# ADVRHumanoids/OpenSoT

Measured on AMD Instinct MI355X. Metric: whole-body QP solves/sec (32-DoF, 3-level stack), higher is better.
Workload: dtype f64

## Files before the change

opensot_amd/csrc/osot_host_plan.h:

```cpp
#pragma once
#include "osot_plan_shape.h"
#include "osot_kernels.h"

namespace osot {

inline int pick_np(int n) {
#ifdef OSOT_X_NO_NP40
    return (n <= 32) ? 32 : ((n <= WaveCtx<56>::NMAX) ? 56 : 64);
#else
    return (n <= 32) ? 32 : ((n <= WaveCtx<40>::NMAX) ? 40 : ((n <= WaveCtx<56>::NMAX) ? 56 : 64));
#endif
}
inline int wave_lds_doubles(int NP) {
    return NP == 32 ? WaveCtx<32>::LDS_DOUBLES : (NP == 40 ? WaveCtx<40>::LDS_DOUBLES : (NP == 56 ? WaveCtx<56>::LDS_DOUBLES : WaveCtx<64>::LDS_DOUBLES));
}

inline int lds_layout(int NP, int n_rows, int* rows_off, int* rows_cap) {
    int d = (wave_lds_doubles(NP) + 1) & ~1;
    *rows_off = d;
    const int cap = ((n_rows > 0 ? n_rows : 1) + 1) & ~1;
    *rows_cap = cap;
    d += row_table_doubles(cap);
    d = (d + 1) & ~1;
    return d;
}

inline int make_dev_plan(const osot_plan_desc& p, const unsigned char* level_active, DevPlan& P, int& NP,
                         size_t& lds_bytes, const unsigned char* task_active = nullptr) {
    std::memset(&P, 0, sizeof(P));
    make_plan_shape(p, level_active, task_active, P);
    for (int k = 0; k < p.n_levels; ++k) P.ident_rows[k] = P.m[k] - P.ma[k];
    NP = pick_np(p.n);
    const int nrows_max = P.nc + P.optoff[p.n_levels];
    const int cap = ((nrows_max > 0 ? nrows_max : 1) + 1) & ~1;
    int total = (wave_lds_doubles(NP) + 1) & ~1;
    P.lds_rows_off = total;
    P.lds_rows_cap = cap;
    const int table = row_table_doubles(cap);
    P.rows_doubles = table;
    P.rows_in_global = 0;
    if (NP > 32) {
        const size_t with = (size_t)(total + table) * sizeof(double), without = (size_t)total * sizeof(double);
        if ((160 * 1024) / without > (160 * 1024) / with) P.rows_in_global = 1;
    }
    if (!P.rows_in_global) total += table;
    lds_bytes = (size_t)total * sizeof(double);
    return OSOT_OK;
}

inline void make_update_plan(const osot_plan_desc& pl, DevUpdatePlan& U) {
    std::memset(&U, 0, sizeof(U));
    U.n = pl.n; U.L = pl.n_levels;
    plan_constraint_rows(&pl, &U.nc);
    plan_stored_constraint_rows(&pl, &U.nc_stored);
    int flat = 0;
    for (int k = 0; k < pl.n_levels; ++k) {
        plan_level_rows(&pl, k, &U.m[k], &U.ma[k]);
        int off = 0;
        for (int j = 0; j < pl.level[k].n_tasks; ++j) {
            const osot_task_desc& t = pl.level[k].task[j];
            DevTaskS& d = U.task[flat++];
            d.level = k; d.kind = t.kind; d.rows = t.rows; d.off = off;
            d.weight = t.weight; d.lambda = t.lambda; d.ogain = t.orientation_gain; d.lambda2 = t.lambda2;
            d.mask = t.row_mask; d.prow = task_parent_rows(t, pl.n); d.sublam = t.row_mask ? t.sub_lambda : 1.0;
            d.gains = t.acc_gain_matrices ? 1 : 0;
            d.body = t.body_frame; d.dense = t.dense_weight;
            if (t.dense_weight) U.dense_level[k] = 1;
            off += t.rows;
        }
    }
    if (pl.has_regularisation) {
        const osot_task_desc& t = pl.regularisation;
        DevTaskS& d = U.task[flat++];
        d.level = -1; d.kind = t.kind; d.rows = t.rows; d.off = 0;
        d.weight = t.weight; d.lambda = t.lambda; d.ogain = t.orientation_gain; d.lambda2 = t.lambda2;
        d.mask = 0ull; d.prow = t.rows; d.sublam = 1.0;
        d.gains = 0; d.body = 0; d.dense = 0;
    }
    U.ntasks = flat;
    {
        int fr = 0;
        for (int j = 0; j < flat; ++j)
            for (int r = 0; r < U.task[j].rows && fr < OSOT_KMAX_FLAT_ROWS; ++r, ++fr) { U.row_task[fr] = (unsigned char)j; U.row_in_task[fr] = (short)r; }
        U.total_rows = fr;
        for (int k = 0; k < pl.n_levels; ++k) if (U.dense_level[k]) U.any_dense = 1;
    }
    U.nbounds = pl.n_bounds;
    for (int j = 0; j < pl.n_bounds; ++j) {
        U.bound[j].kind = pl.bound[j].kind; U.bound[j].scaling = pl.bound[j].scaling; U.bound[j].dT = pl.bound[j].dT;
    }
    U.nrowblocks = pl.n_rowblocks;
    int roff = 0, soff = 0;
    for (int j = 0; j < pl.n_rowblocks; ++j) {
        const osot_rows_desc& r = pl.rowblock[j];
        DevRowBlockS& d = U.rowblock[j];
        d.kind = r.kind; d.rows = r.rows; d.off = roff; d.stored_off = soff; d.first_col = r.first_col;
        d.body = r.task_body_frame; d.ncand = r.n_candidates;
        d.dT = r.dT; d.p = r.p; d.mu = r.mu; d.lambda = r.task_lambda; d.ogain = r.task_orientation_gain;
        for (int i = 0; i < OSOT_MAX_BAND_ROWS; ++i) { d.err_lb[i] = r.err_lb[i]; d.err_ub[i] = r.err_ub[i]; }
        d.d_threshold = r.d_threshold; d.detection_threshold = r.detection_threshold; d.bound_scaling = r.bound_scaling;
        if (!rows_are_implicit(d.kind)) soff += d.rows;
        roff += d.rows;
    }
}

inline int make_update_args(const osot_plan_desc& pl, const DevUpdatePlan& PL, const osot_leaf_batch* leaf,
                            const osot_assembled_out* out, const DevUpdatePlan* dev_plan, DevUpdate& U, const char** why) {
    std::memset(&U, 0, sizeof(U));
    U.B = leaf->B;
    U.plan = dev_plan;
    int flat = 0;
    for (int k = 0; k < pl.n_levels; ++k) {
        if (!out->b[k]) { *why = "out.b[k] is null"; return OSOT_ERR_INVALID; }
        U.b[k] = out->b[k]; U.w[k] = out->w[k];
        if (PL.dense_level[k]) {
            if (!out->WA[k] || !out->Wb[k] || (PL.ma[k] > 0 && !out->A[k]))
                { *why = "level has a non-diagonal weight: out.WA[k], out.Wb[k] and out.A[k] are required"; return OSOT_ERR_INVALID; }
            U.WA[k] = out->WA[k]; U.Wb[k] = out->Wb[k]; U.A[k] = out->A[k];
        }
        for (int j = 0; j < pl.level[k].n_tasks; ++j) {
            const osot_task_desc& t = pl.level[k].task[j];
            DevPtr4& d = U.task[flat++];
            d.p0 = leaf->task[k][j].p0; d.p1 = leaf->task[k][j].p1; d.p2 = leaf->task[k][j].p2; d.W = leaf->task[k][j].W;
            if (!d.p0) { *why = "leaf input p0 of a task is null"; return OSOT_ERR_INVALID; }
            if (t.kind != OSOT_TASK_GENERIC && t.kind != OSOT_TASK_ACC_POSTURAL && !d.p1)
                { *why = "leaf input p1 of a task is null"; return OSOT_ERR_INVALID; }
            if (t.dense_weight && !d.W) { *why = "task has dense_weight but its leaf W is null"; return OSOT_ERR_INVALID; }
        }
    }
    if (pl.has_regularisation) {
        const osot_task_desc& t = pl.regularisation;
        if (!out->b_reg) { *why = "out.b_reg is null"; return OSOT_ERR_INVALID; }
        DevPtr4& d = U.task[flat++];
        d.p0 = leaf->regularisation.p0; d.p1 = leaf->regularisation.p1; d.p2 = leaf->regularisation.p2; d.W = nullptr;
        if (!d.p0) { *why = "leaf input p0 of the regularisation task is null"; return OSOT_ERR_INVALID; }
        if (t.kind == OSOT_TASK_POSTURAL && !d.p1) { *why = "leaf input p1 of the regularisation task is null"; return OSOT_ERR_INVALID; }
        U.b_reg = out->b_reg;
    }
    for (int j = 0; j < pl.n_bounds; ++j) {
        DevPtr3& d = U.bound[j];
        const int kind = pl.bound[j].kind;
        d.p0 = leaf->bound[j].p0; d.p1 = leaf->bound[j].p1; d.p2 = leaf->bound[j].p2;
        if (!d.p0) { *why = "leaf input p0 of a bound is null"; return OSOT_ERR_INVALID; }
        if (kind == OSOT_BOUND_JOINT_LIMITS && (!d.p1 || !d.p2)) { *why = "joint limits need q, q_min, q_max"; return OSOT_ERR_INVALID; }
        if (kind == OSOT_BOUND_GENERIC && !d.p1) { *why = "generic bound needs l and u"; return OSOT_ERR_INVALID; }
    }
    if (pl.n_bounds > 0 && (!out->l || !out->u)) { *why = "out.l/out.u is null"; return OSOT_ERR_INVALID; }
    U.l = out->l; U.u = out->u;
    for (int j = 0; j < pl.n_rowblocks; ++j) {
        DevPtr3& d = U.rows[j];
        const int kind = pl.rowblock[j].kind;
        d.p0 = leaf->rows[j].p0; d.p1 = leaf->rows[j].p1; d.p2 = leaf->rows[j].p2;
        if (!d.p0) { *why = "leaf input p0 of a row block is null"; return OSOT_ERR_INVALID; }
        if ((kind == OSOT_ROWS_GENERIC || kind == OSOT_ROWS_COLLISION || kind == OSOT_ROWS_TORQUE_LIMITS ||
             kind == OSOT_ROWS_ACC_JOINT_LIMITS || kind == OSOT_ROWS_ACC_VELOCITY_LIMITS ||
             kind == OSOT_ROWS_TASK_CARTESIAN || kind == OSOT_ROWS_TASK_COM || kind == OSOT_ROWS_UNIT_GENERIC) && !d.p1)
            { *why = "leaf input p1 of a row block is null"; return OSOT_ERR_INVALID; }
        if (kind == OSOT_ROWS_ACC_JOINT_LIMITS && !d.p2) { *why = "acceleration joint limits need qddot_max"; return OSOT_ERR_INVALID; }
        if (kind == OSOT_ROWS_GENERIC && !d.p2) { *why = "generic rows need C, lo, up"; return OSOT_ERR_INVALID; }
        if ((kind == OSOT_ROWS_COP || kind == OSOT_ROWS_NORMAL_TORQUE) && !d.p1)
            { *why = "CoP / normal torque rows need the contact's x / y limits (p1)"; return OSOT_ERR_INVALID; }
    }
    if (PL.nc > 0 && (!out->lo || !out->up)) { *why = "out.lo/up is null"; return OSOT_ERR_INVALID; }
    if (PL.nc_stored > 0 && !out->C) { *why = "out.C is null"; return OSOT_ERR_INVALID; }
    U.C = out->C; U.lo = out->lo; U.up = out->up;
    return OSOT_OK;
}

}
```

opensot_amd/csrc/osot_kernels.h:

```cpp
#pragma once
#include "osot_plan_shape.h"
#include "osot_qp_core.h"

#ifndef OSOT_WAVES32
#define OSOT_WAVES32 2
#endif
#ifndef OSOT_WAVES40
#define OSOT_WAVES40 2
#endif

namespace osot {

struct DevPlan {
    int n, L, nc;
    int m[OSOT_KMAX_LEVELS];
    int ma[OSOT_KMAX_LEVELS];
    int optoff[OSOT_KMAX_LEVELS + 1];
    int ident_rows[OSOT_KMAX_LEVELS];
    int nblocks, nc_stored;
    int blk_rows[OSOT_KMAX_ROWBLOCKS], blk_off[OSOT_KMAX_ROWBLOCKS], blk_stored_off[OSOT_KMAX_ROWBLOCKS];
    int blk_implicit[OSOT_KMAX_ROWBLOCKS], blk_first_col[OSOT_KMAX_ROWBLOCKS];
    int blk_level[OSOT_KMAX_ROWBLOCKS];
    int max_iter;
    unsigned active_mask;
    int ntask[OSOT_KMAX_LEVELS];
    int task_off[OSOT_KMAX_LEVELS][OSOT_KMAX_TASKS + 1];
    unsigned inactive[OSOT_KMAX_LEVELS];
    double eps_abs;
    int reg_rows;
    double reg_w;
    int reg_dense;
    int lds_rows_off;
    int lds_rows_cap;
    int rows_doubles;
    int rows_in_global;
};

struct DevBatch {
    int B;
    const double* A[OSOT_KMAX_LEVELS];
    const double* b[OSOT_KMAX_LEVELS];
    const double* w[OSOT_KMAX_LEVELS];
    const double* c[OSOT_KMAX_LEVELS];
    const double* C;
    const double* lo;
    const double* up;
    const double* l;
    const double* u;
    double* dq;
    double* x_levels;
    int* status;
    int* iterations;
    long long* prof;
    const int* order;
    int* cost_out;
    const int* cost_in;
    int* order_next;
    int slots;
    const double* b_reg;
    const double* A_reg;
    const double* WA[OSOT_KMAX_LEVELS];
    const double* Wb[OSOT_KMAX_LEVELS];
    double* accepted_slack;
    double* rows_scratch;
    int* hot;
};
static_assert(std::is_trivially_copyable<DevPlan>::value && std::is_trivially_copyable<DevBatch>::value, "kernel arguments, zeroed with memset");

template <int NP, bool PROF, bool EXTRA, bool BOX = false>
__device__ __forceinline__ void cascade_body(const DevPlan& P, const DevBatch& D, const long long inst, const int lane, char* osot_smem) {
    constexpr int HV = WaveCtx<NP>::HV, S = WaveCtx<NP>::S;
    constexpr int HB = (NP % 16 == 0) ? 16 : 8;
    const int n = P.n;
    double* base = reinterpret_cast<double*>(osot_smem);
    WaveCtx<NP> w;
    w.c = WaveCtx<NP>::col_of(lane); w.h = WaveCtx<NP>::half_of(lane); w.n = n;
    w.M1 = base;
    w.M2 = base + WaveCtx<NP>::M1_DOUBLES;
    w.V = w.M2 + WaveCtx<NP>::ROWS * S;
    if constexpr (NP == 32) w.rlo = base + P.lds_rows_off;
    else w.rlo = P.rows_in_global ? D.rows_scratch + inst * P.rows_doubles : base + P.lds_rows_off;
    w.rup = w.rlo + P.lds_rows_cap;
    w.rptr = reinterpret_cast<unsigned long long*>(w.rup + P.lds_rows_cap);
    w.rowstate = reinterpret_cast<int*>(w.rptr + P.lds_rows_cap);
    w.eqlist = w.rowstate + P.lds_rows_cap;
    w.safe_row = reinterpret_cast<unsigned long long>(D.dq + inst * n);
    w.rsrc = reinterpret_cast<signed char*>(w.eqlist + P.lds_rows_cap);
    const int c = w.c, h = w.h;
    const bool valid = c < n;
    for (int e = lane; e < WaveCtx<NP>::LDS_DOUBLES; e += 64) base[e] = 0.0;
    wave_sync();

    const bool has_box = D.l != nullptr;
    double lb = (has_box && valid) ? D.l[inst * n + c] : -INFINITY;
    double ub = (has_box && valid) ? D.u[inst * n + c] : INFINITY;

    for (int j = 0; j < P.nblocks; ++j) {
        for (int q = lane; q < P.blk_rows[j]; q += 64) {
            const int r = P.blk_off[j] + q;
            w.rlo[r] = clamp_inf(D.lo[inst * P.nc + r]);
            w.rup[r] = clamp_inf(D.up[inst * P.nc + r]);
            w.rptr[r] = P.blk_implicit[j]
                ? ((((unsigned long long)(P.blk_first_col[j] + q)) << 1) | 1ull)
                : reinterpret_cast<unsigned long long>(D.C + (inst * P.nc_stored + P.blk_stored_off[j] + q) * n);
            w.rsrc[r] = -1;
        }
    }
    wave_sync();

    const bool regd = EXTRA && P.reg_dense && D.b_reg != nullptr;
    const bool regc = D.b_reg != nullptr && !regd && c < P.reg_rows;
    const double greg = regc ? -P.reg_w * D.b_reg[inst * P.reg_rows + c] : 0.0;
    const double dreg = regc ? P.reg_w : 0.0;

    double x = 0.0;
    int status = QP_SOLVED;
    int iters_total = 0;
    bool any = false;
    double slack = 0.0;
    long long prof[PH_COUNT];
    if (PROF) for (int i = 0; i < PH_COUNT; ++i) prof[i] = 0;
    const long long t_begin = PROF ? (long long)clock64() : 0;
    for (int k = 0; k < P.L; ++k) {
        if (!((P.active_mask >> k) & 1u)) {
            if (k + 1 < P.L) {
                const int off = P.nc + P.optoff[k];
                for (int q = lane; q < P.m[k]; q += 64) {
                    w.rlo[off + q] = -kInfty; w.rup[off + q] = kInfty; w.rptr[off + q] = (0x7fffffffull << 1) | 1ull;
                    w.rsrc[off + q] = -1;
                }
                wave_sync();
            }
            continue;
        }
        for (int j = 0; j < P.nblocks; ++j) {
            if (P.blk_level[j] == 0) continue;
            const bool on = P.blk_level[j] - 1 == k;
            for (int q = lane; q < P.blk_rows[j]; q += 64) {
                const int r = P.blk_off[j] + q;
                w.rlo[r] = on ? clamp_inf(D.lo[inst * P.nc + r]) : -kInfty;
                w.rup[r] = on ? clamp_inf(D.up[inst * P.nc + r]) : kInfty;
                w.rsrc[r] = on ? -2 : -1;
            }
            wave_sync();
        }
        OSOT_PH_BEGIN();
        {
            const int l2 = launder_i(lane);
            w.c = WaveCtx<NP>::col_of(l2); w.h = WaveCtx<NP>::half_of(l2);
        }
        const int c = w.c, h = w.h;
        const bool valid = c < n;
        const int m = P.m[k], ma = P.ma[k];
// ... 456 lines not shown
    const int h0 = hist[4 * lane], h1 = hist[4 * lane + 1], h2 = hist[4 * lane + 2], h3 = hist[4 * lane + 3];
    const int tot = h0 + h1 + h2 + h3;
    int v = tot;
#pragma unroll
    for (int off = 1; off < 64; off <<= 1) {
        const int t = __shfl_down(v, off, 64);
        v += (lane + off < 64) ? t : 0;
    }
    const int above = v - tot;
    start[4 * lane + 3] = above;
    start[4 * lane + 2] = above + h3;
    start[4 * lane + 1] = above + h3 + h2;
    start[4 * lane] = above + h3 + h2 + h1;
    __syncthreads();
    const int late = B - slots;
    const bool paired = late > 0 && B < 2 * slots;
    for (int i = lane; i < B; i += 64) {
        const int pos = __hip_atomic_fetch_add(&start[key(i)], 1, __ATOMIC_RELAXED, __HIP_MEMORY_SCOPE_WORKGROUP);
        int where = pos;
        if (paired) {
            const int alone = slots - late;
            if (pos >= B - late) where = alone + (B - 1 - pos);
            else if (pos >= alone) where = slots + (pos - alone);
        }
        order[where] = i;
    }
}
#else
inline void order_body(const int*, int*, int, int, int, char*) {}
#endif

__device__ __forceinline__ long long dispatch_instance(const DevBatch& D, char* smem) {
    int g = (int)blockIdx.x;
    if (D.order_next) {
        if (g == 0) { order_body(D.cost_in, D.order_next, D.B, D.slots, (int)threadIdx.x, smem); return -1; }
        g -= 1;
    }
    if (D.order) wave_priority_by_rank((unsigned)g, (unsigned)D.B);
    return D.order ? D.order[g] : g;
}

struct DevQP {
    int B, n, nc, max_iter;
    double eps_abs;
    const double* H;
    const double* g;
    const double* A;
    const double* lA;
    const double* uA;
    const double* l;
    const double* u;
    double* x;
    int* status;
    int* iterations;
    int lds_rows_off, lds_rows_cap;
    int* hot;
};

template <int NP, bool HOT = false>
__global__ void __launch_bounds__(64, (NP == 40 ? OSOT_WAVES40 : 1)) osot_qp_kernel(const DevQP Q) {
    OSOT_DYNAMIC_LDS(osot_smem);
    constexpr int S = WaveCtx<NP>::S;
    const int lane = threadIdx.x;
    const long long inst = blockIdx.x;
    const int n = Q.n;
    double* base = reinterpret_cast<double*>(osot_smem);
    WaveCtx<NP> w;
    w.c = WaveCtx<NP>::col_of(lane); w.h = WaveCtx<NP>::half_of(lane); w.n = n;
    w.M1 = base; w.M2 = base + WaveCtx<NP>::M1_DOUBLES; w.V = w.M2 + WaveCtx<NP>::ROWS * S;
    w.rlo = base + Q.lds_rows_off;
    w.rup = w.rlo + Q.lds_rows_cap;
    w.rptr = reinterpret_cast<unsigned long long*>(w.rup + Q.lds_rows_cap);
    w.rowstate = reinterpret_cast<int*>(w.rptr + Q.lds_rows_cap);
    w.eqlist = w.rowstate + Q.lds_rows_cap;
    w.safe_row = reinterpret_cast<unsigned long long>(Q.x + inst * n);
    w.rsrc = reinterpret_cast<signed char*>(w.eqlist + Q.lds_rows_cap);
    const int c = w.c, h = w.h;
    const bool valid = c < n;
    for (int e = lane; e < WaveCtx<NP>::LDS_DOUBLES; e += 64) base[e] = 0.0;
    wave_sync();
    constexpr int HV = WaveCtx<NP>::HV;
    double Hc[NP / HV];
    if constexpr (NP == 32) {
        const int ta = lane & 15, tq = lane >> 4;
#pragma unroll
        for (int t = 0; t < 16; ++t) {
            const int i = 16 * (t >> 3) + tq + 4 * (t & 3), cc = 16 * ((t >> 2) & 1) + ta;
            Hc[t] = (i < n && cc < n) ? Q.H[(inst * n + i) * n + cc] + ((i == cc) ? Q.eps_abs : 0.0)
                                      : ((i == cc) ? 1.0 : 0.0);
        }
    } else if constexpr (kWideTiles) {
        constexpr int T = wide_tiles(NP);
        const int ta = lane & 15, tq = lane >> 4;
#pragma unroll
        for (int I = 0; I < T; ++I)
#pragma unroll
            for (int C2 = I; C2 < T; ++C2)
#pragma unroll
                for (int r = 0; r < 4; ++r) {
                    const int i = 16 * I + tq + 4 * r, cc = 16 * C2 + ta;
                    Hc[4 * tile_u<T>(I, C2) + r] = (i < n && cc < n) ? Q.H[(inst * n + i) * n + cc] + ((i == cc) ? Q.eps_abs : 0.0)
                                                                      : ((i == cc) ? 1.0 : 0.0);
                }
    } else {
#pragma unroll
        for (int ii = 0; ii < NP / HV; ++ii) {
            const int i = HV * ii + h;
            Hc[ii] = (valid && i < n) ? Q.H[(inst * n + i) * n + c] + ((i == c) ? Q.eps_abs : 0.0)
                                      : ((i == c) ? 1.0 : 0.0);
        }
    }
    wave_sync();
    const double g = valid ? Q.g[inst * n + c] : 0.0;
    const bool has_box = Q.l != nullptr;
    double lb = (has_box && valid) ? Q.l[inst * n + c] : -INFINITY;
    double ub = (has_box && valid) ? Q.u[inst * n + c] : INFINITY;
    for (int r = lane; r < Q.nc; r += 64) {
        w.rlo[r] = clamp_inf(Q.lA[inst * Q.nc + r]);
        w.rup[r] = clamp_inf(Q.uA[inst * Q.nc + r]);
        w.rptr[r] = reinterpret_cast<unsigned long long>(Q.A + (inst * Q.nc + r) * n);
        w.rsrc[r] = -1;
    }
    wave_sync();
    double x = 0.0, slack = 0.0;
    int iters = 0;
    int st;
    int* hotk = (HOT && Q.hot) ? Q.hot + inst * WaveCtx<NP>::LW : nullptr;
    const int hotcode = hotk ? hotk[c] : -1;
    if (NP > 32) {
        OSOT_ALWAYS_INLINE_CALL st = gi_solve<NP, false>(w, Q.nc, g, false, 0.0, Hc, has_box, lb, ub, Q.max_iter, false, 0.0, x, iters, nullptr, slack,
                                                         false, 0.0, hotcode, hotk);
    } else {
        st = gi_solve<NP, false>(w, Q.nc, g, false, 0.0, Hc, has_box, lb, ub, Q.max_iter, false, 0.0, x, iters, nullptr, slack,
                                 false, 0.0, hotcode, hotk);
    }
    if (valid && h == 0) Q.x[inst * n + c] = (st == QP_SOLVED) ? x : 0.0;
    if (lane == 0) {
        Q.status[inst] = st;
        if (Q.iterations) Q.iterations[inst] = iters;
    }
}

struct DevTaskS {
    int level, kind, rows, off, prow, body, dense, gains;
    double weight, lambda, ogain, lambda2, sublam;
    unsigned long long mask;
};
struct DevBoundS { int kind; double scaling, dT; };
struct DevRowBlockS {
    int kind, rows, off, stored_off, first_col, body, ncand;
    double d_threshold, detection_threshold, bound_scaling, dT, p, mu, lambda, ogain;
    double err_lb[OSOT_MAX_BAND_ROWS], err_ub[OSOT_MAX_BAND_ROWS];
};
struct DevUpdatePlan {
    int n, L, nc, nc_stored;
    int m[OSOT_KMAX_LEVELS], ma[OSOT_KMAX_LEVELS];
    int dense_level[OSOT_KMAX_LEVELS];
    int any_dense;
    int total_rows;
    unsigned char row_task[OSOT_KMAX_FLAT_ROWS];
    short row_in_task[OSOT_KMAX_FLAT_ROWS];
    int ntasks;
    DevTaskS task[OSOT_KMAX_FLAT_TASKS];
    int nbounds;
    DevBoundS bound[OSOT_KMAX_BOUNDS];
    int nrowblocks;
    DevRowBlockS rowblock[OSOT_KMAX_ROWBLOCKS];
};
struct DevPtr4 { const double *p0, *p1, *p2, *W; };
struct DevPtr3 { const double *p0, *p1, *p2; };
struct DevUpdate {
    int B;
    const DevUpdatePlan* plan;
    DevPtr4 task[OSOT_KMAX_FLAT_TASKS];
    DevPtr3 bound[OSOT_KMAX_BOUNDS];
    DevPtr3 rows[OSOT_KMAX_ROWBLOCKS];
    double* b[OSOT_KMAX_LEVELS];
    double* w[OSOT_KMAX_LEVELS];
    double* WA[OSOT_KMAX_LEVELS];
    double* Wb[OSOT_KMAX_LEVELS];
    const double* A[OSOT_KMAX_LEVELS];
    double* C;
    double* lo;
    double* up;
    double* l;
    double* u;
    double* b_reg;
};
static_assert(sizeof(DevUpdate) <= 4096, "kernel arguments are limited to 4 KB");
static_assert(sizeof(DevUpdate) % 16 == 0 && sizeof(DevUpdatePlan) % 16 == 0, "staged into LDS in 16-byte pieces");
constexpr int kUpdateLdsBytes = (int)sizeof(DevUpdate) + (int)sizeof(DevUpdatePlan) + 256 * 8 + 258 * 4 + 8;

__device__ inline void rot_to_quat(const double* R, double* q) {
    double t = R[0] + R[4] + R[8];
    if (t > 0.0) {
        t = sqrt(t + 1.0);
        q[3] = 0.5 * t;
        t = 0.5 / t;
        q[0] = (R[7] - R[5]) * t;
        q[1] = (R[2] - R[6]) * t;
        q[2] = (R[3] - R[1]) * t;
    } else {
        int i = 0;
        if (R[4] > R[0]) i = 1;
        if (R[8] > ((i == 1) ? R[4] : R[0])) i = 2;
        if (i == 0) {
            t = sqrt(R[0] - R[4] - R[8] + 1.0);
            q[0] = 0.5 * t;
            t = 0.5 / t;
            q[3] = (R[7] - R[5]) * t;
            q[1] = (R[3] + R[1]) * t;
            q[2] = (R[6] + R[2]) * t;
        } else if (i == 1) {
            t = sqrt(R[4] - R[8] - R[0] + 1.0);
            q[1] = 0.5 * t;
            t = 0.5 / t;
            q[3] = (R[2] - R[6]) * t;
            q[2] = (R[7] + R[5]) * t;
            q[0] = (R[1] + R[3]) * t;
        } else {
            t = sqrt(R[8] - R[0] - R[4] + 1.0);
            q[2] = 0.5 * t;
            t = 0.5 / t;
            q[3] = (R[3] - R[1]) * t;
            q[0] = (R[2] + R[6]) * t;
            q[1] = (R[5] + R[7]) * t;
        }
    }
}

__device__ inline void cartesian_b(const double* Ta, const double* Td, const double* twist,
                                   double lambda, double ogain, double* b6, bool body = false) {
    double q[4], qd[4];
    rot_to_quat(Ta, q);
    rot_to_quat(Td, qd);
    const double dot = q[0] * qd[0] + q[1] * qd[1] + q[2] * qd[2] + q[3] * qd[3];
    const double sg = (dot < 0.0) ? -1.0 : 1.0;
    const double qx = sg * q[0], qy = sg * q[1], qz = sg * q[2], qw = sg * q[3];
    double eo[3];
    eo[0] = qd[3] * qx - qw * qd[0] + (-qd[2] * qy + qd[1] * qz);
    eo[1] = qd[3] * qy - qw * qd[1] + (qd[2] * qx - qd[0] * qz);
    eo[2] = qd[3] * qz - qw * qd[2] + (-qd[1] * qx + qd[0] * qy);
    for (int i = 0; i < 3; ++i) {
        const double tw_p = twist ? twist[i] : 0.0, tw_o = twist ? twist[3 + i] : 0.0;
        b6[i] = tw_p + lambda * (Td[9 + i] - Ta[9 + i]);
        b6[3 + i] = tw_o + lambda * (-ogain * eo[i]);
    }
    if (body) {
        double r6[6];
        for (int i = 0; i < 3; ++i) {
            r6[i] = Ta[i] * b6[0] + Ta[3 + i] * b6[1] + Ta[6 + i] * b6[2];
            r6[3 + i] = Ta[i] * b6[3] + Ta[3 + i] * b6[4] + Ta[6 + i] * b6[5];
        }
        for (int i = 0; i < 6; ++i) b6[i] = r6[i];
    }
}

__device__ inline double wrench_row_entry(int kind, int rr, int col, const double* R, const double* lim, double mu) {
    double a[6] = {0.0, 0.0, 0.0, 0.0, 0.0, 0.0};
    if (kind == 10) {
        const double m = mu / sqrt(2.0);
        a[0] = (rr == 0) ? 1.0 : (rr == 1 ? -1.0 : 0.0);
        a[1] = (rr == 2) ? 1.0 : (rr == 3 ? -1.0 : 0.0);
        a[2] = (rr == 4) ? -1.0 : -m;
    } else if (kind == 11) {
        const double xl = lim[0], xu = lim[1], yl = lim[2], yu = lim[3];
        a[2] = rr == 0 ? xl : (rr == 1 ? -xu : (rr == 2 ? yl : -yu));
        a[3] = rr == 2 ? -1.0 : (rr == 3 ? 1.0 : 0.0);
        a[4] = rr == 0 ? 1.0 : (rr == 1 ? -1.0 : 0.0);
    } else {
        const double xl = lim[0], xu = lim[1], yl = lim[2], yu = lim[3];
        const double X = (fabs(xl) + fabs(xu)) / 2., Y = (fabs(yl) + fabs(yu)) / 2.;
        const double px = (xu + xl) / 2., py = (yu + yl) / 2.;
        const double K = -mu * (X + Y);
        const double sy = (rr == 0 || rr == 1 || rr == 6 || rr == 7) ? -1.0 : 1.0;
        const double sx = (rr == 0 || rr == 2 || rr == 5 || rr == 7) ? -1.0 : 1.0;
        const double sa = (rr == 0 || rr == 1 || rr == 4 || rr == 5) ? -1.0 : 1.0;
        const double sb = (rr == 0 || rr == 2 || rr == 4 || rr == 6) ? -1.0 : 1.0;
        const double sz = rr < 4 ? 1.0 : -1.0;
        const double a0 = sy * Y, a1 = sx * X, a3 = sa * mu, a4 = sb * mu;
        a[0] = a0 - sz * py;
        a[1] = a1 + sz * px;
        a[2] = K + a3 * py - a4 * px;
        a[3] = a3; a[4] = a4; a[5] = sz;
    }
    const int o = col < 3 ? 0 : 3, c = col < 3 ? col : col - 3;
    return a[o] * R[c * 3 + 0] + a[o + 1] * R[c * 3 + 1] + a[o + 2] * R[c * 3 + 2];
}

__device__ __forceinline__ void update_body(const DevUpdate* args_global, const long long inst, const int t, char* lds) {
    DevUpdate* Ul = reinterpret_cast<DevUpdate*>(lds);
    DevUpdatePlan* Pl = reinterpret_cast<DevUpdatePlan*>(lds + sizeof(DevUpdate));
    double* dcand = reinterpret_cast<double*>(lds + sizeof(DevUpdate) + sizeof(DevUpdatePlan));
    int* src_of_row = reinterpret_cast<int*>(dcand + 256);
    int* n_used_s = src_of_row + 256;
    {
        struct alignas(16) v2f64 { double a, b; };
        constexpr int NA = (int)sizeof(DevUpdate) / 16, NP_ = (int)sizeof(DevUpdatePlan) / 16;
        const v2f64* ga = reinterpret_cast<const v2f64*>(args_global);
        const v2f64* gp = reinterpret_cast<const v2f64*>(args_global->plan);
        v2f64* la = reinterpret_cast<v2f64*>(Ul);
        v2f64* lp = reinterpret_cast<v2f64*>(Pl);
        v2f64 va[(NA + 63) / 64], vp[(NP_ + 63) / 64];
#pragma unroll
        for (int i = 0; i < (NA + 63) / 64; ++i) { const int e = t + 64 * i; va[i] = ga[e < NA ? e : 0]; }
#pragma unroll
        for (int i = 0; i < (NP_ + 63) / 64; ++i) { const int e = t + 64 * i; vp[i] = gp[e < NP_ ? e : 0]; }
#pragma unroll
        for (int i = 0; i < (NA + 63) / 64; ++i) { const int e = t + 64 * i; if (e < NA) la[e] = va[i]; }
#pragma unroll
        for (int i = 0; i < (NP_ + 63) / 64; ++i) { const int e = t + 64 * i; if (e < NP_) lp[e] = vp[i]; }
        wave_sync();
    }
    const DevUpdate& U = *Ul;
    const DevUpdatePlan& PL = *Pl;
    const int n = PL.n;
    for (int fr = t; fr < PL.total_rows; fr += 64) {
        const int j = PL.row_task[fr], r = PL.row_in_task[fr];
        const DevTaskS& tk = PL.task[j];
        const int kind = tk.kind, level = tk.level, prow = tk.prow;
        const unsigned long long mask = tk.mask;
        const double *p0 = U.task[j].p0, *p1 = U.task[j].p1, *p2 = U.task[j].p2;
        double* bl;
        double* wl = nullptr;
        if (level < 0) bl = U.b_reg + inst * tk.rows + r;
        else {
            bl = U.b[level] + inst * PL.m[level] + tk.off + r;
            if (U.w[level]) wl = U.w[level] + inst * PL.m[level] + tk.off + r;
        }
        if (wl) *wl = tk.weight;
        if (kind == 1) continue;
        const bool acc = (kind == 4 || kind == 5 || kind == 6);
        int pr = r;
        if (mask != 0ull) {
            unsigned long long mm = mask;
            for (int q = 0; q < r; ++q) mm &= mm - 1ull;
            pr = __builtin_ctzll(mm);
        }
        const long long base = inst * (long long)prow + pr;
        double x0, x1;
        if (acc && tk.gains) {
            const double* e = p0 + inst * (2LL * prow + 2LL * prow * prow);
            const double* Gp = e + 2 * prow + pr * prow;
            const double* Gd = Gp + prow * prow;
            double ap = 0.0, ad = 0.0;
            for (int q = 0; q < prow; ++q) { ap = fma(Gp[q], e[q], ap); ad = fma(Gd[q], e[prow + q], ad); }
            x0 = ap; x1 = ad;
        } else {
            x0 = acc ? p0[inst * 2LL * prow + pr] : p0[base];
            x1 = acc ? p0[inst * 2LL * prow + prow + pr] : 0.0;
        }
        const double x2 = (p1 && kind != 0 && kind != 6) ? p1[base] : 0.0;
        const double x3 = (p2 && kind != 0) ? p2[base] : 0.0;
        const double lam = tk.lambda, lam2 = tk.lambda2;
        double v;
        if (kind == 2 || kind == 3) {
            v = x3 + lam * (x2 - x0);
        } else if (kind == 4 || kind == 5) {
            v = x3 + lam2 * x1 + lam * x0 - x2;
        } else if (kind == 6) {
            v = x3 + lam2 * x1 + lam * x0;
        } else {
            v = x0;
        }
        *bl = (mask != 0ull) ? v * tk.sublam : v;
    }
    if (t < PL.ntasks && PL.task[t].kind == 1) {
        const DevTaskS& tk = PL.task[t];
        const double *cp0 = U.task[t].p0, *cp1 = U.task[t].p1, *cp2 = U.task[t].p2;
        double* cb = (tk.level < 0) ? U.b_reg + inst * tk.rows
                                    : U.b[tk.level] + inst * PL.m[tk.level] + tk.off;
        const unsigned cmask = (tk.mask != 0ull) ? ((unsigned)tk.mask & 0x3fu) : 0x3fu;
        const double csub = (tk.mask != 0ull) ? tk.sublam : 1.0;
        double Ta[12], Td[12], tw[6], b6[6];
#pragma unroll
        for (int i = 0; i < 12; ++i) { Ta[i] = cp0[inst * 12 + i]; Td[i] = cp1[inst * 12 + i]; }
#pragma unroll
        for (int i = 0; i < 6; ++i) tw[i] = cp2 ? cp2[inst * 6 + i] : 0.0;
        cartesian_b(Ta, Td, tw, tk.lambda, tk.ogain, b6, tk.body != 0);
        int kq = 0;
#pragma unroll
        for (int i = 0; i < 6; ++i) if ((cmask >> i) & 1u) { cb[kq] = b6[i] * csub; kq++; }
    }
    {
        if (PL.any_dense) {
            workgroup_fence();
            __syncthreads();
            for (int j = 0; j < PL.ntasks; ++j) {
                const DevTaskS& tk = PL.task[j];
                if (tk.level < 0 || !PL.dense_level[tk.level]) continue;
                const int k = tk.level, mk = PL.m[k], mak = PL.ma[k];
                const double* bk = U.b[k] + inst * mk + tk.off;
                double* wbk = U.Wb[k] + inst * mk + tk.off;
                const bool stored = tk.off + tk.rows <= mak;
                const double* Ak = stored ? U.A[k] + (inst * mak + tk.off) * n : nullptr;
                double* WAk = stored ? U.WA[k] + (inst * mak + tk.off) * n : nullptr;
                const double* Wm = tk.dense ? U.task[j].W + inst * tk.rows * tk.rows : nullptr;
                for (int r = 0; r < tk.rows; ++r) {
                    if (Wm) {
                        double wb = 0.0;
                        for (int q = 0; q < tk.rows; ++q) wb = fma(Wm[r * tk.rows + q], bk[q], wb);
                        if (t == 0) wbk[r] = tk.weight * wb;
                        for (int c0 = t; c0 < n; c0 += 64) {
                            double acc = 0.0;
                            for (int q = 0; q < tk.rows; ++q) acc = fma(Wm[r * tk.rows + q], Ak[q * n + c0], acc);
                            WAk[r * n + c0] = tk.weight * acc;
                        }
                    } else {
                        if (t == 0) wbk[r] = tk.weight * bk[r];
                        if (stored) for (int c0 = t; c0 < n; c0 += 64) WAk[r * n + c0] = tk.weight * Ak[r * n + c0];
                    }
                }
            }
        }
    }
    if (PL.nbounds > 0) {
        for (int i = t; i < n; i += 64) {
            double l = 0.0, u = 0.0;
            for (int j = 0; j < PL.nbounds; ++j) {
                const DevBoundS& bd = PL.bound[j];
                const DevPtr3& bp = U.bound[j];
                double l2, u2;
                if (bd.kind == 1) {
                    const double q = bp.p0[inst * n + i];
                    u2 = fmax((bp.p2[inst * n + i] - q) * bd.scaling, 0.0);
                    l2 = fmin((bp.p1[inst * n + i] - q) * bd.scaling, 0.0);
                } else if (bd.kind == 2) {
                    const double v = fabs(bp.p0[inst * n + i]) * bd.dT;
                    l2 = -1.0 * v; u2 = 1.0 * v;
                } else { l2 = bp.p0[inst * n + i]; u2 = bp.p1[inst * n + i]; }
                if (j == 0) { l = l2; u = u2; } else { u = fmin(u, u2); l = fmax(l, l2); }
            }
            U.l[inst * n + i] = l;
            U.u[inst * n + i] = u;
        }
    }
    for (int j = 0; j < PL.nrowblocks; ++j) {
        const DevRowBlockS& rb = PL.rowblock[j];
        const DevPtr3& rp = U.rows[j];
        double* Cb = U.C ? U.C + (inst * PL.nc_stored + rb.stored_off) * n : nullptr;
        double* lob = U.lo + inst * PL.nc + rb.off;
        double* upb = U.up + inst * PL.nc + rb.off;
        if (rb.kind == 1) {
            const int ncand = rb.ncand > 0 ? rb.ncand : rb.rows;
            const double* Jd = rp.p0 + inst * ncand * n;
            const double* dist = rp.p1 + inst * ncand;
            int& n_used = n_used_s[0];
            for (int i = t; i < ncand; i += 64) {
                const double d = dist[i];
                dcand[i] = (rb.detection_threshold > 0 && d > rb.detection_threshold) ? INFINITY : d;
            }
            for (int i = t; i < 256; i += 64) src_of_row[i] = -1;
            __syncthreads();
            int mine_used = 0;
            for (int i = t; i < ncand; i += 64) {
                const double d = dcand[i];
                if (d < INFINITY) {
                    int rank = 0;
                    for (int q = 0; q < ncand; ++q) { const double dq = dcand[q]; rank += (dq < d || (dq == d && q < i)) ? 1 : 0; }
                    if (rank < rb.rows) src_of_row[rank] = i;
                    mine_used++;
                }
            }
            (void)mine_used;
            if (t == 0) {
                int cnt = 0;
                for (int q = 0; q < ncand; ++q) cnt += (dcand[q] < INFINITY) ? 1 : 0;
                n_used = cnt;
            }
            __syncthreads();
            const int nu = n_used < rb.rows ? n_used : rb.rows;
            for (int r = 0; r < rb.rows; ++r) {
                const bool used = r < nu;
                const int src = used ? src_of_row[r] : 0;
                for (int i = t; i < n; i += 64) Cb[r * n + i] = used ? -Jd[src * n + i] : 0.0;
                if (t == 0) {
                    if (used) {
                        const double ub = rb.bound_scaling * (dist[src] - rb.d_threshold);
                        upb[r] = ub < 0.0 ? 0.0 : ub;
                    } else upb[r] = 1.7976931348623157e308;
                    lob[r] = -1.7976931348623157e308;
                }
            }
            __syncthreads();
        } else if (rb.kind == 9) {
            for (int r = t; r < rb.rows; r += 64) { lob[r] = rp.p0[inst * rb.rows + r]; upb[r] = rp.p1[inst * rb.rows + r]; }
        } else if (rb.kind == 7) {
            if (t == 0) {
                double Ta[12], Td[12], tw[6], b6[6];
#pragma unroll
                for (int i = 0; i < 12; ++i) { Ta[i] = rp.p0[inst * 12 + i]; Td[i] = rp.p1[inst * 12 + i]; }
#pragma unroll
                for (int i = 0; i < 6; ++i) tw[i] = rp.p2 ? rp.p2[inst * 6 + i] : 0.0;
                cartesian_b(Ta, Td, tw, rb.lambda, rb.ogain, b6, rb.body != 0);
                for (int i = 0; i < 6; ++i) { lob[i] = b6[i] + rb.err_lb[i]; upb[i] = b6[i] + rb.err_ub[i]; }
            }
        } else if (rb.kind == 8) {
            if (t < 3) {
                const double b = (rp.p2 ? rp.p2[inst * 3 + t] : 0.0) + rb.lambda * (rp.p1[inst * 3 + t] - rp.p0[inst * 3 + t]);
                lob[t] = b + rb.err_lb[t]; upb[t] = b + rb.err_ub[t];
            }
        } else if (rb.kind == 2) {
            if (t < 6) { const double v = -rp.p0[inst * 6 + t]; lob[t] = v; upb[t] = v; }
        } else if (rb.kind == 3) {
            for (int r = t; r < rb.rows; r += 64) {
                const double hh = rp.p0[inst * rb.rows + r], tm = rp.p1[inst * rb.rows + r];
                lob[r] = -tm - hh; upb[r] = tm - hh;
            }
        } else if (rb.kind == 4) {
            const int nct = rb.rows / 5;
            const double mu = rb.mu / sqrt(2.0);
            for (int e = t; e < rb.rows * n; e += 64) Cb[e] = 0.0;
            __syncthreads();
            for (int e = t; e < nct * 15; e += 64) {
                const int ct = e / 15, rr = (e % 15) / 3, col = e % 3;
                const double* R = rp.p0 + (inst * nct + ct) * 9;
                const double ci0 = (rr == 0) ? 1.0 : (rr == 1 ? -1.0 : 0.0);
                const double ci1 = (rr == 2) ? 1.0 : (rr == 3 ? -1.0 : 0.0);
                const double ci2 = (rr == 4) ? -1.0 : -mu;
                Cb[(ct * 5 + rr) * n + rb.first_col + ct * 3 + col] = ci0 * R[col * 3 + 0] + ci1 * R[col * 3 + 1] + ci2 * R[col * 3 + 2];
            }
            for (int r = t; r < rb.rows; r += 64) { lob[r] = -1.0e20; upb[r] = 0.0; }
        } else if (rb.kind >= 10 && rb.kind <= 12) {
            const int per = rb.kind == 10 ? 5 : (rb.kind == 11 ? 4 : 8);
            const int nct = rb.rows / per;
            for (int e = t; e < rb.rows * n; e += 64) Cb[e] = 0.0;
            __syncthreads();
            for (int e = t; e < nct * per * 6; e += 64) {
                const int ct = e / (per * 6), rr = (e / 6) % per, col = e % 6;
                const double* R = rp.p0 + (inst * nct + ct) * 9;
                const double* lim = rb.kind == 10 ? nullptr : rp.p1 + (inst * nct + ct) * 4;
                Cb[(ct * per + rr) * n + rb.first_col + ct * 6 + col] = wrench_row_entry(rb.kind, rr, col, R, lim, rb.mu);
            }
            for (int r = t; r < rb.rows; r += 64) { lob[r] = -1.0e20; upb[r] = 0.0; }
        } else if (rb.kind == 5) {
            const int nr = rb.rows;
            const double dt = rb.dT * rb.p;
            for (int i = t; i < nr; i += 64) {
                const double q = rp.p0[inst * 2 * nr + i], qd = rp.p0[inst * 2 * nr + nr + i];
                const double qmin = rp.p1[inst * 2 * nr + i], qmax = rp.p1[inst * 2 * nr + nr + i];
                const double am = rp.p2[inst * nr + i];
                const double a = .5 * dt * dt / am;
                const double b_sup = dt * qd / am + .5 * dt * dt;
                const double c_sup = q + dt * qd - qmax + .5 * qd * qd / am;
                double delta_sup = b_sup * b_sup - 4 * a * c_sup;
                const double b_inf = dt * qd / am - .5 * dt * dt;
                const double c_inf = -q - dt * qd + qmin + .5 * qd * qd / am;
                double delta_inf = b_inf * b_inf - 4 * a * c_inf;
                if (delta_sup < 0) delta_sup = 0;
                if (delta_inf < 0) delta_inf = 0;
                const double ub_sup = .5 / a * (-b_sup + sqrt(delta_sup)), lb_sup = .5 / a * (-b_sup - sqrt(delta_sup));
                const double ub_inf = .5 / a * (-b_inf + sqrt(delta_inf)), lb_inf = .5 / a * (-b_inf - sqrt(delta_inf));
                double ub = fmin(ub_sup, ub_inf);
                const double lb = fmax(lb_sup, lb_inf);
                if (ub < lb) ub = lb;
                lob[i] = lb; upb[i] = ub;
            }
        } else if (rb.kind == 6) {
            for (int i = t; i < rb.rows; i += 64) {
                const double qd = rp.p0[inst * rb.rows + i], lim = rp.p1[inst * rb.rows + i];
                upb[i] = (lim - qd) / (rb.dT * rb.p);
                lob[i] = (-lim - qd) / (rb.dT * rb.p);
            }
        } else {
            for (int e = t; e < rb.rows * n; e += 64) Cb[e] = rp.p0[inst * rb.rows * n + e];
            for (int r = t; r < rb.rows; r += 64) { lob[r] = rp.p1[inst * rb.rows + r]; upb[r] = rp.p2[inst * rb.rows + r]; }
        }
    }
}

__global__ void __launch_bounds__(64) osot_update_kernel(const DevUpdate U) {
    OSOT_STATIC_LDS(double, upd_lds, kUpdateLdsBytes / 8);
    if ((long long)blockIdx.x >= U.B) return;
    update_body(OSOT_KERNARG_PTR(DevUpdate, U), blockIdx.x, threadIdx.x, reinterpret_cast<char*>(upd_lds));
}

template <int NP, bool EXTRA = false, bool BOX = false>
__global__ void __launch_bounds__(64, (NP == 32 ? OSOT_WAVES32 : (NP == 40 ? OSOT_WAVES40 : 1))) osot_cycle_kernel(const DevUpdate U, const DevPlan P, const DevBatch D) {
    OSOT_DYNAMIC_LDS(osot_smem);
    const long long inst = dispatch_instance(D, osot_smem);
    if (inst < 0) return;
    const long long tc0 = D.prof ? (long long)clock64() : 0;
    const long long tw0 = D.prof ? (long long)wall_clock64() : 0;
    update_body(OSOT_KERNARG_PTR(DevUpdate, U), inst, (int)threadIdx.x, osot_smem);
    workgroup_fence();
    __syncthreads();
    const long long tc1 = D.prof ? (long long)clock64() : 0;
    cascade_body<NP, false, EXTRA, BOX>(P, D, inst, (int)threadIdx.x, osot_smem);
    if (D.prof && threadIdx.x == 0) {
// ... 9 lines not shown
```

Before: 34.00 million.

## Replace LDS staging of update args with precomputed per-row records and lane permutes

Removes the per-block copy of the whole DevUpdate argument block and update plan into LDS. Instead, the host precomputes one 64-byte record per flat row and per cartesian task, and each lane fetches its own pointers from the kernel arguments, with other lanes' pointers obtained through wave permutes. The first row's leaf loads, the cartesian input loads and the bounds computation are reordered so their global loads can overlap. LDS use drops to the scratch buffers, which may raise occupancy, at the cost of more complex slot mapping and larger plan structs in global memory.

Result: no change. 34.22 million, median of 6 (+0.7%).

```diff
diff --git a/opensot_amd/csrc/osot_host_plan.h b/opensot_amd/csrc/osot_host_plan.h
--- a/opensot_amd/csrc/osot_host_plan.h
+++ b/opensot_amd/csrc/osot_host_plan.h
@@ -46,6 +46,61 @@
     if (!P.rows_in_global) total += table;
     lds_bytes = (size_t)total * sizeof(double);
     return OSOT_OK;
+}
+
+inline int upd_slot_of(size_t off) {
+    const int w = (int)(off / 8);
+    if (w >= kUpdSlotTask && w < kUpdSlotTask + 64) return w - kUpdSlotTask;
+    for (int lane = 0; lane <= 48; ++lane) if (upd_slot_word1(lane) == w) return 64 + lane;
+    return -1;
+}
+inline size_t upd_slot_offset(int slot) { return 8 * (size_t)(slot < 64 ? kUpdSlotTask + slot : upd_slot_word1(slot - 64)); }
+
+inline void make_update_table(DevUpdatePlan& U) {
+    for (int i = 0; i < OSOT_KMAX_FLAT_ROWS; ++i) U.row_rec[i].kind = -1;
+    for (int i = 0; i < OSOT_KMAX_FLAT_TASKS; ++i) U.cart_rec[i].kind = -1;
+    const auto fill = [&](DevUpdRec& d, int j) {
+        const DevTaskS& tk = U.task[j];
+        d.kind = (signed char)tk.kind;
+        d.prow = tk.prow;
+        const bool acc = tk.kind == 4 || tk.kind == 5 || tk.kind == 6;
+        d.flags = (unsigned char)((acc ? kUpdRecAcc : 0u) | (tk.gains ? kUpdRecGains : 0u) | (tk.mask != 0ull ? kUpdRecMasked : 0u) |
+                                  (tk.body ? kUpdRecBody : 0u));
+        d.s_p0 = (unsigned char)upd_slot_of(offsetof(DevUpdate, task) + sizeof(DevPtr4) * j + offsetof(DevPtr4, p0));
+        d.s_p1 = (unsigned char)upd_slot_of(offsetof(DevUpdate, task) + sizeof(DevPtr4) * j + offsetof(DevPtr4, p1));
+        d.s_p2 = (unsigned char)upd_slot_of(offsetof(DevUpdate, task) + sizeof(DevPtr4) * j + offsetof(DevPtr4, p2));
+        if (tk.level < 0) {
+            d.s_b = (unsigned char)upd_slot_of(offsetof(DevUpdate, b_reg));
+            d.s_w = (unsigned char)kUpdSlotNone;
+            d.out_stride = tk.rows; d.out_off = 0;
+        } else {
+            d.s_b = (unsigned char)upd_slot_of(offsetof(DevUpdate, b) + sizeof(double*) * tk.level);
+            d.s_w = (unsigned char)upd_slot_of(offsetof(DevUpdate, w) + sizeof(double*) * tk.level);
+            d.out_stride = U.m[tk.level]; d.out_off = tk.off;
+        }
+        d.lambda = tk.lambda; d.lambda2 = tk.lambda2; d.weight = tk.weight; d.sublam = tk.sublam;
+    };
+    for (int fr = 0; fr < U.total_rows; ++fr) {
+        const int j = U.row_task[fr], r = U.row_in_task[fr];
+        DevUpdRec& d = U.row_rec[fr];
+        fill(d, j);
+        d.out_off += r;
+        d.pr = r;
+        if (U.task[j].mask != 0ull) {
+            unsigned long long mm = U.task[j].mask;
+            for (int q = 0; q < r; ++q) mm &= mm - 1ull;
+            d.pr = __builtin_ctzll(mm);
+        }
+    }
+    int nc = 0;
+    for (int j = 0; j < U.ntasks; ++j) {
+        if (U.task[j].kind != 1) continue;
+        DevUpdRec& d = U.cart_rec[nc++];
+        fill(d, j);
+        d.pr = (U.task[j].mask != 0ull) ? (int)((unsigned)U.task[j].mask & 0x3fu) : 0x3f;
+        d.lambda2 = U.task[j].ogain;
+        d.sublam = (U.task[j].mask != 0ull) ? U.task[j].sublam : 1.0;
+    }
 }
 
 inline void make_update_plan(const osot_plan_desc& pl, DevUpdatePlan& U) {
@@ -102,6 +157,7 @@
         if (!rows_are_implicit(d.kind)) soff += d.rows;
         roff += d.rows;
     }
+    make_update_table(U);
 }
 
 inline int make_update_args(const osot_plan_desc& pl, const DevUpdatePlan& PL, const osot_leaf_batch* leaf,
diff --git a/opensot_amd/csrc/osot_kernels.h b/opensot_amd/csrc/osot_kernels.h
--- a/opensot_amd/csrc/osot_kernels.h
+++ b/opensot_amd/csrc/osot_kernels.h
@@ -1,4 +1,5 @@
 #pragma once
+#include <cstddef>
 #include "osot_plan_shape.h"
 #include "osot_qp_core.h"
 
@@ -761,6 +762,21 @@
     double d_threshold, detection_threshold, bound_scaling, dT, p, mu, lambda, ogain;
     double err_lb[OSOT_MAX_BAND_ROWS], err_ub[OSOT_MAX_BAND_ROWS];
 };
+struct alignas(16) DevUpdRec {
+    int prow;
+    int pr;
+    int out_stride;
+    int out_off;
+    signed char kind;
+    unsigned char flags;
+    unsigned char s_p0, s_p1, s_p2, s_b, s_w;
+    unsigned char pad0;
+    double lambda, lambda2, weight, sublam;
+    double pad1;
+};
+static_assert(sizeof(DevUpdRec) == 64, "one record = four 16-byte loads");
+constexpr unsigned kUpdRecAcc = 1u, kUpdRecGains = 2u, kUpdRecMasked = 4u, kUpdRecBody = 8u;
+constexpr int kUpdSlotNone = 255;
 struct DevUpdatePlan {
     int n, L, nc, nc_stored;
     int m[OSOT_KMAX_LEVELS], ma[OSOT_KMAX_LEVELS];
@@ -775,6 +791,8 @@
     DevBoundS bound[OSOT_KMAX_BOUNDS];
     int nrowblocks;
     DevRowBlockS rowblock[OSOT_KMAX_ROWBLOCKS];
+    DevUpdRec row_rec[OSOT_KMAX_FLAT_ROWS];
+    DevUpdRec cart_rec[OSOT_KMAX_FLAT_TASKS];
 };
 struct DevPtr4 { const double *p0, *p1, *p2, *W; };
 struct DevPtr3 { const double *p0, *p1, *p2; };
@@ -797,8 +815,15 @@
     double* b_reg;
 };
 static_assert(sizeof(DevUpdate) <= 4096, "kernel arguments are limited to 4 KB");
-static_assert(sizeof(DevUpdate) % 16 == 0 && sizeof(DevUpdatePlan) % 16 == 0, "staged into LDS in 16-byte pieces");
-constexpr int kUpdateLdsBytes = (int)sizeof(DevUpdate) + (int)sizeof(DevUpdatePlan) + 256 * 8 + 258 * 4 + 8;
+constexpr int kUpdSlotTask = (int)(offsetof(DevUpdate, task) / 8);
+constexpr int kUpdSlotB = (int)(offsetof(DevUpdate, b) / 8);
+constexpr int kUpdSlotW = (int)(offsetof(DevUpdate, w) / 8);
+constexpr int kUpdSlotReg = (int)(offsetof(DevUpdate, b_reg) / 8);
+static_assert(4 * OSOT_KMAX_FLAT_TASKS == 96 && OSOT_KMAX_LEVELS == 8 && kUpdSlotW == kUpdSlotB + 8, "the slot layout above");
+__host__ __device__ inline int upd_slot_word1(int lane) {
+    return lane < 32 ? kUpdSlotTask + 64 + lane : (lane < 48 ? kUpdSlotB + (lane - 32) : kUpdSlotReg);
+}
+constexpr int kUpdateLdsBytes = 256 * 8 + 258 * 4 + 8;
 
 __device__ inline void rot_to_quat(const double* R, double* q) {
     double t = R[0] + R[4] + R[8];
@@ -897,71 +922,63 @@
     return a[o] * R[c * 3 + 0] + a[o + 1] * R[c * 3 + 1] + a[o + 2] * R[c * 3 + 2];
 }
 
+__device__ __forceinline__ const double* upd_slot_ptr(int slot, double w0, double w1) {
+    const int a4 = (slot & 63) << 2;
+    const double a = permute_f64(w0, a4), b = permute_f64(w1, a4);
+    const double v = (slot & 64) ? b : a;
+    unsigned long long bits;
+    __builtin_memcpy(&bits, &v, 8);
+    return slot == kUpdSlotNone ? nullptr : reinterpret_cast<const double*>(bits);
+}
+struct UpdRowLeaves { double x0, x1, x2, x3; double* bl; };
+
 __device__ __forceinline__ void update_body(const DevUpdate* args_global, const long long inst, const int t, char* lds) {
-    DevUpdate* Ul = reinterpret_cast<DevUpdate*>(lds);
-    DevUpdatePlan* Pl = reinterpret_cast<DevUpdatePlan*>(lds + sizeof(DevUpdate));
-    double* dcand = reinterpret_cast<double*>(lds + sizeof(DevUpdate) + sizeof(DevUpdatePlan));
+    double* dcand = reinterpret_cast<double*>(lds);
     int* src_of_row = reinterpret_cast<int*>(dcand + 256);
     int* n_used_s = src_of_row + 256;
-    {
-        struct alignas(16) v2f64 { double a, b; };
-        constexpr int NA = (int)sizeof(DevUpdate) / 16, NP_ = (int)sizeof(DevUpdatePlan) / 16;
-        const v2f64* ga = reinterpret_cast<const v2f64*>(args_global);
-        const v2f64* gp = reinterpret_cast<const v2f64*>(args_global->plan);
-        v2f64* la = reinterpret_cast<v2f64*>(Ul);
-        v2f64* lp = reinterpret_cast<v2f64*>(Pl);
-        v2f64 va[(NA + 63) / 64], vp[(NP_ + 63) / 64];
-#pragma unroll
-        for (int i = 0; i < (NA + 63) / 64; ++i) { const int e = t + 64 * i; va[i] = ga[e < NA ? e : 0]; }
-#pragma unroll
-        for (int i = 0; i < (NP_ + 63) / 64; ++i) { const int e = t + 64 * i; vp[i] = gp[e < NP_ ? e : 0]; }
-#pragma unroll
-        for (int i = 0; i < (NA + 63) / 64; ++i) { const int e = t + 64 * i; if (e < NA) la[e] = va[i]; }
-#pragma unroll
-        for (int i = 0; i < (NP_ + 63) / 64; ++i) { const int e = t + 64 * i; if (e < NP_) lp[e] = vp[i]; }
-        wave_sync();
-    }
-    const DevUpdate& U = *Ul;
-    const DevUpdatePlan& PL = *Pl;
-    const int n = PL.n;
-    for (int fr = t; fr < PL.total_rows; fr += 64) {
-        const int j = PL.row_task[fr], r = PL.row_in_task[fr];
-        const DevTaskS& tk = PL.task[j];
-        const int kind = tk.kind, level = tk.level, prow = tk.prow;
-        const unsigned long long mask = tk.mask;
-        const double *p0 = U.task[j].p0, *p1 = U.task[j].p1, *p2 = U.task[j].p2;
-        double* bl;
-        double* wl = nullptr;
-        if (level < 0) bl = U.b_reg + inst * tk.rows + r;
-        else {
-            bl = U.b[level] + inst * PL.m[level] + tk.off + r;
-            if (U.w[level]) wl = U.w[level] + inst * PL.m[level] + tk.off + r;
-        }
-        if (wl) *wl = tk.weight;
-        if (kind == 1) continue;
-        const bool acc = (kind == 4 || kind == 5 || kind == 6);
-        int pr = r;
-        if (mask != 0ull) {
-            unsigned long long mm = mask;
-            for (int q = 0; q < r; ++q) mm &= mm - 1ull;
-            pr = __builtin_ctzll(mm);
-        }
+    const DevUpdate& U = *args_global;
+    const DevUpdatePlan& PL = *U.plan;
+    const double* words = reinterpret_cast<const double*>(args_global);
+    const double w0 = words[kUpdSlotTask + t];
+    const double w1 = words[upd_slot_word1(t)];
+    const DevUpdRec rec0 = PL.row_rec[t];
+    const DevUpdRec crec = PL.cart_rec[t < OSOT_KMAX_FLAT_TASKS ? t : 0];
+    const bool is_cart = t < OSOT_KMAX_FLAT_TASKS && crec.kind == 1;
+    const int n = PL.n, total_rows = PL.total_rows;
+    auto row_issue = [&](const DevUpdRec& rc, UpdRowLeaves& v) {
+        const double *p0 = upd_slot_ptr(rc.s_p0, w0, w1), *p1 = upd_slot_ptr(rc.s_p1, w0, w1), *p2 = upd_slot_ptr(rc.s_p2, w0, w1);
+        double* bo = const_cast<double*>(upd_slot_ptr(rc.s_b, w0, w1));
+        double* wo = const_cast<double*>(upd_slot_ptr(rc.s_w, w0, w1));
+        v.x0 = v.x1 = v.x2 = v.x3 = 0.0;
+        v.bl = nullptr;
+        const int kind = rc.kind;
+        if (kind < 0) return;
+        const long long oo = inst * rc.out_stride + rc.out_off;
+        if (wo) wo[oo] = rc.weight;
+        if (kind == 1) return;
+        v.bl = bo + oo;
+        const bool acc = (rc.flags & kUpdRecAcc) != 0;
+        const int prow = rc.prow, pr = rc.pr;
         const long long base = inst * (long long)prow + pr;
-        double x0, x1;
-        if (acc && tk.gains) {
+        if (acc && (rc.flags & kUpdRecGains)) {
             const double* e = p0 + inst * (2LL * prow + 2LL * prow * prow);
             const double* Gp = e + 2 * prow + pr * prow;
             const double* Gd = Gp + prow * prow;
             double ap = 0.0, ad = 0.0;
             for (int q = 0; q < prow; ++q) { ap = fma(Gp[q], e[q], ap); ad = fma(Gd[q], e[prow + q], ad); }
-            x0 = ap; x1 = ad;
+            v.x0 = ap; v.x1 = ad;
         } else {
-            x0 = acc ? p0[inst * 2LL * prow + pr] : p0[base];
-            x1 = acc ? p0[inst * 2LL * prow + prow + pr] : 0.0;
-        }
-        const double x2 = (p1 && kind != 0 && kind != 6) ? p1[base] : 0.0;
-        const double x3 = (p2 && kind != 0) ? p2[base] : 0.0;
-        const double lam = tk.lambda, lam2 = tk.lambda2;
+            v.x0 = acc ? p0[inst * 2LL * prow + pr] : p0[base];
+            v.x1 = acc ? p0[inst * 2LL * prow + prow + pr] : 0.0;
+        }
+        v.x2 = (p1 && kind != 0 && kind != 6) ? p1[base] : 0.0;
+        v.x3 = (p2 && kind != 0) ? p2[base] : 0.0;
+    };
+    auto row_finish = [&](const DevUpdRec& rc, const UpdRowLeaves& lv) {
+        if (!lv.bl) return;
+        const int kind = rc.kind;
+        const double x0 = lv.x0, x1 = lv.x1, x2 = lv.x2, x3 = lv.x3;
+        const double lam = rc.lambda, lam2 = rc.lambda2;
         double v;
         if (kind == 2 || kind == 3) {
             v = x3 + lam * (x2 - x0);
@@ -972,24 +989,56 @@
         } else {
             v = x0;
         }
-        *bl = (mask != 0ull) ? v * tk.sublam : v;
-    }
-    if (t < PL.ntasks && PL.task[t].kind == 1) {
-        const DevTaskS& tk = PL.task[t];
-        const double *cp0 = U.task[t].p0, *cp1 = U.task[t].p1, *cp2 = U.task[t].p2;
-        double* cb = (tk.level < 0) ? U.b_reg + inst * tk.rows
-                                    : U.b[tk.level] + inst * PL.m[tk.level] + tk.off;
-        const unsigned cmask = (tk.mask != 0ull) ? ((unsigned)tk.mask & 0x3fu) : 0x3fu;
-        const double csub = (tk.mask != 0ull) ? tk.sublam : 1.0;
-        double Ta[12], Td[12], tw[6], b6[6];
+        *lv.bl = (rc.flags & kUpdRecMasked) ? v * rc.sublam : v;
+    };
+    UpdRowLeaves lv0;
+    row_issue(rec0, lv0);
+    const double *cp0 = upd_slot_ptr(crec.s_p0, w0, w1), *cp1 = upd_slot_ptr(crec.s_p1, w0, w1), *cp2 = upd_slot_ptr(crec.s_p2, w0, w1);
+    double* cb = const_cast<double*>(upd_slot_ptr(crec.s_b, w0, w1));
+    double Ta[12], Td[12], tw[6];
+    if (is_cart) {
 #pragma unroll
         for (int i = 0; i < 12; ++i) { Ta[i] = cp0[inst * 12 + i]; Td[i] = cp1[inst * 12 + i]; }
 #pragma unroll
         for (int i = 0; i < 6; ++i) tw[i] = cp2 ? cp2[inst * 6 + i] : 0.0;
-        cartesian_b(Ta, Td, tw, tk.lambda, tk.ogain, b6, tk.body != 0);
+    }
+    if (PL.nbounds > 0) {
+        for (int i = t; i < n; i += 64) {
+            double l = 0.0, u = 0.0;
+            for (int j = 0; j < PL.nbounds; ++j) {
+                const DevBoundS& bd = PL.bound[j];
+                const DevPtr3& bp = U.bound[j];
+                double l2, u2;
+                if (bd.kind == 1) {
+                    const double q = bp.p0[inst * n + i];
+                    u2 = fmax((bp.p2[inst * n + i] - q) * bd.scaling, 0.0);
+                    l2 = fmin((bp.p1[inst * n + i] - q) * bd.scaling, 0.0);
+                } else if (bd.kind == 2) {
+                    const double v = fabs(bp.p0[inst * n + i]) * bd.dT;
+                    l2 = -1.0 * v; u2 = 1.0 * v;
+                } else { l2 = bp.p0[inst * n + i]; u2 = bp.p1[inst * n + i]; }
+                if (j == 0) { l = l2; u = u2; } else { u = fmin(u, u2); l = fmax(l, l2); }
+            }
+            U.l[inst * n + i] = l;
+            U.u[inst * n + i] = u;
+        }
+    }
+    row_finish(rec0, lv0);
+    if (is_cart) {
+        const unsigned cmask = (unsigned)crec.pr;
+        const double csub = crec.sublam;
+        double b6[6];
+        cartesian_b(Ta, Td, tw, crec.lambda, crec.lambda2, b6, (crec.flags & kUpdRecBody) != 0);
+        cb += inst * crec.out_stride + crec.out_off;
         int kq = 0;
 #pragma unroll
         for (int i = 0; i < 6; ++i) if ((cmask >> i) & 1u) { cb[kq] = b6[i] * csub; kq++; }
+    }
+    for (int f0 = 64; f0 < total_rows; f0 += 64) {
+        const DevUpdRec rc = PL.row_rec[f0 + t];
+        UpdRowLeaves lv;
+        row_issue(rc, lv);
+        row_finish(rc, lv);
     }
     {
         if (PL.any_dense) {
@@ -1023,27 +1072,6 @@
             }
         }
     }
-    if (PL.nbounds > 0) {
-        for (int i = t; i < n; i += 64) {
-            double l = 0.0, u = 0.0;
-            for (int j = 0; j < PL.nbounds; ++j) {
-                const DevBoundS& bd = PL.bound[j];
-                const DevPtr3& bp = U.bound[j];
-                double l2, u2;
-                if (bd.kind == 1) {
-                    const double q = bp.p0[inst * n + i];
-                    u2 = fmax((bp.p2[inst * n + i] - q) * bd.scaling, 0.0);
-                    l2 = fmin((bp.p1[inst * n + i] - q) * bd.scaling, 0.0);
-                } else if (bd.kind == 2) {
-                    const double v = fabs(bp.p0[inst * n + i]) * bd.dT;
-                    l2 = -1.0 * v; u2 = 1.0 * v;
-                } else { l2 = bp.p0[inst * n + i]; u2 = bp.p1[inst * n + i]; }
-                if (j == 0) { l = l2; u = u2; } else { u = fmin(u, u2); l = fmax(l, l2); }
-            }
-            U.l[inst * n + i] = l;
-            U.u[inst * n + i] = u;
-        }
-    }
     for (int j = 0; j < PL.nrowblocks; ++j) {
         const DevRowBlockS& rb = PL.rowblock[j];
         const DevPtr3& rp = U.rows[j];
```
